# jspenmar/slowtv_monodepth

Hardware: AMD Instinct MI355X
Metric: training images/sec (640×192, 3-frame) at 1/2/4/8 MI355X; warp+SSIM HBM GB/s (higher is better)
Workload: dtype f32

## Files before the change

### slowtv_monodepth_amd/csrc/smd_conv_mfma.hip

```cpp
#include "smd_common.h"
#include "smd_kernels.h"
#include "smd_conv_mfma_dev.h"
#include <algorithm>

namespace smd {

template <typename T> __device__ __forceinline__ void store_out(T* p, size_t i, float v);
template <> __device__ __forceinline__ void store_out<float>(float* p, size_t i, float v) { p[i] = v; }
template <> __device__ __forceinline__ void store_out<bf16>(bf16* p, size_t i, float v) { p[i] = __float2bfloat16(v); }

template <int P>
__global__ __launch_bounds__(256) void k_conv_pack_w(const float* __restrict__ w, unsigned short* __restrict__ wp_fwd, unsigned short* __restrict__ wp_bwd, int CO, int C) {
  const int idx = blockIdx.x*256 + threadIdx.x;
  if (idx >= CO*C*9) return;
  const int tap = idx % 9, c = (idx/9) % C, co = idx/(9*C);
  unsigned pk[P];
  split_pair<P>(w[idx], 0.f, pk);
  if (wp_fwd) {
    const size_t base = ((((size_t)(co >> 5)*(C >> 4) + (c >> 4))*9 + tap)*P)*512 + (((c >> 3) & 1)*32 + (co & 31))*8 + (c & 7);
#pragma unroll
    for (int p = 0; p < P; ++p) wp_fwd[base + (size_t)p*512] = (unsigned short)(pk[p] & 0xffffu);
  }
  if (wp_bwd) {
    const size_t base = ((((size_t)(c >> 5)*(CO >> 4) + (co >> 4))*9 + (8 - tap))*P)*512 + (((co >> 3) & 1)*32 + (c & 31))*8 + (co & 7);
#pragma unroll
    for (int p = 0; p < P; ++p) wp_bwd[base + (size_t)p*512] = (unsigned short)(pk[p] & 0xffffu);
  }
}

#ifdef SMD_CONV_TRACE
__device__ unsigned long long g_conv_trace[8192][40];
#define SMD_CT(slot) do { if (wall == 0 && lid < 8192u && (slot) < 40) { const unsigned long long t_ = __builtin_amdgcn_s_memtime(); if (lane == 0) g_conv_trace[lid][(slot)] = t_; } } while (0)
#else
#define SMD_CT(slot) do { } while (0)
#endif
template <int TC> struct ConvTile {
  static constexpr int TRB = (TC == 64) ? 4 : 8;
  static constexpr int PW = TC + 2, PH = TRB + 2, NPIX = PW*PH;
};
template <> struct ConvTile<0> {
  static constexpr int TRB = 0, PW = 0, NPIX = 420;
};

template <int TC, int P, int OFF, typename TI, typename TO, int NM>
__global__ __launch_bounds__(256*NM, 2/NM) void k_conv_mfma(const TI* __restrict__ in_, const uint4* __restrict__ wp, TO* __restrict__ out,
                                                   int CK, int M, int hi, int wi, int ho, int wo, int KS, int kc_per_split, size_t split_stride,
                                                   unsigned gx, unsigned gy, unsigned gz, int S, int B) {
  using T = ConvTile<TC>;
  constexpr bool BAND = TC == 0;
  constexpr int NPIX = T::NPIX, off = OFF;
  const int PW = BAND ? wo + 2 : T::PW;
  constexpr bool ZERO = OFF != 0;
  constexpr int kBuf = P*NPIX*2;
  __shared__ uint4 tile[2*kBuf];
  const int lane = threadIdx.x & 63, wall = __builtin_amdgcn_readfirstlane(threadIdx.x >> 6), wv = wall & 3, mt = wall >> 2, j = lane & 31, g = lane >> 5;
  constexpr int NT = 256*NM;
  const int MG = M/(32*NM);
  const unsigned nblk = (unsigned)(MG*KS)*(BAND ? 1u : gx)*gy*gz, lid = xcd_block_id(nblk);
  if (lid >= nblk) return;
  const int mg = (int)(lid % MG)*NM + mt, ks = (lid/MG) % KS;
  const unsigned tl = lid/(MG*KS);
  const int BR = BAND ? (int)gx : 0, SEGP = (BR + 2)*PW;
  const int x0 = BAND ? 0 : (int)(tl % gx)*TC, y0 = BAND ? (int)(tl % gy)*BR : (int)((tl/gx) % gy)*T::TRB;
  const int b = BAND ? (int)(tl/gy)*S : (int)(tl/(gx*gy));
  const int KC = CK >> 4, kc0 = ks*kc_per_split, kc1 = min(KC, kc0 + kc_per_split);
  const size_t plane = (size_t)hi*wi;
  typedef typename RawOf<TI>::type R;
  const R* src = reinterpret_cast<const R*>(in_) + (size_t)b*CK*plane;
  auto band_pixel = [&](int nt, int& seg, int& ry, int& x) {
    const int p = (2*wv + nt)*32 + j, spx = BR*wo;
    seg = p/spx; const int q = p - seg*spx; ry = q/wo; x = q - ry*wo;
    if (seg >= S || b + seg >= B || y0 + ry >= ho) seg = -1;
  };
  int lbase[2] = {0, 0};
  if constexpr (BAND) {
#pragma unroll
    for (int nt = 0; nt < 2; ++nt) {
      int seg, ry, x;
      band_pixel(nt, seg, ry, x);
      lbase[nt] = seg >= 0 ? (seg*(BR + 2) + ry)*PW + x : 0;
    }
  }

  using Stage = PatchStager<NT, NPIX, P, R, ZERO>;
  constexpr int TRIPS = Stage::TRIPS;
  Stage stage;
  if constexpr (BAND) {
#pragma unroll
    for (int t = 0; t < TRIPS; ++t) {
      const int item = Stage::item(t), half = item >= NPIX ? 1 : 0, pix = item - half*NPIX;
      const int seg = pix/SEGP, rp = pix - seg*SEGP, r = rp/PW, cc = rp - r*PW;
      const int yy = y0 + r - off, xx = cc - off;
      const bool in_b = seg < S && b + seg < B;
      const int sofs = min(seg, B - 1 - b)*CK*(int)plane;
      if (ZERO) stage.pofs[t] = (in_b && yy >= 0 && yy < hi && xx >= 0 && xx < wi) ? sofs + yy*wi + xx : -1;
      else stage.pofs[t] = sofs + min(yy, hi - 1)*wi + min(xx, wi - 1);
    }
  } else stage.template rect_offsets<T::PW>(y0, x0, off, hi, wi);
  R v[TRIPS][8];
  auto request = [&](int kc) { stage.request(src, plane, kc, v); };
  auto file_trip = [&](int buf, int t) { stage.file_trip(tile, buf, t, v); };

  f32x16 acc[2], lo[2];
#pragma unroll
  for (int nt = 0; nt < 2; ++nt)
#pragma unroll
    for (int r = 0; r < 16; ++r) { acc[nt][r] = 0.f; lo[nt][r] = 0.f; }

  bf16x8 A[5][P], Bf[2][2][P];
  const uint4* wq = wp + ((size_t)mg*KC*9*P)*64 + lane;
  auto fetch_a = [&](bf16x8 (&dst)[P], int kc, int tap) {
#pragma unroll
    for (int p = 0; p < P; ++p) dst[p] = as_frag(wq[(size_t)((kc*9 + tap)*P + p)*64]);
  };
  auto read_b = [&](bf16x8 (&dst)[2][P], int buf, int tap) {
    const int ky = tap/3, kx = tap % 3;
#pragma unroll
    for (int nt = 0; nt < 2; ++nt) {
      const int r = (TC == 64) ? wv : 2*wv + nt, cb = (TC == 64) ? nt*32 : 0;
      Stage::read(tile, buf, BAND ? lbase[nt] + ky*PW + kx : (r + ky)*PW + cb + j + kx, g, dst[nt]);
    }
  };
  auto chunk = [&](int kc, int cur, auto more_tag) {
    constexpr bool MORE = decltype(more_tag)::value;
    [[maybe_unused]] const int cslot = 3 + 4*(kc - kc0);
    SMD_CT(cslot);
    read_b(Bf[0], cur, 0);
#pragma unroll
    for (int tap = 0; tap < 9; ++tap) {
      if (tap < 8) read_b(Bf[(tap + 1) & 1], cur, tap + 1);
      split_mfma<P>(A[tap % 5], Bf[tap & 1], acc, lo);
      if (tap <= 4) fetch_a(A[(tap + 4) % 5], kc, tap + 4);
      else if (MORE && tap >= 6) fetch_a(A[tap - 6], kc + 1, tap - 6);
      if (MORE && tap == 8) fetch_a(A[3], kc + 1, 3);
      if (MORE && tap == 4) request(kc + 1);
      if (MORE && tap >= 6) {
#pragma unroll
        for (int t = 0; t < TRIPS; ++t) if (t*3/TRIPS == tap - 6) file_trip(cur ^ 1, t);
      }
      __builtin_amdgcn_sched_barrier(0);
    }
    SMD_CT(cslot + 1);
    SMD_CT(cslot + 2);
    __syncthreads();
    SMD_CT(cslot + 3);
  };

  SMD_CT(0);
  if (kc0 < kc1) {
    request(kc0);
#pragma unroll
    for (int tap = 0; tap < 4; ++tap) fetch_a(A[tap], kc0, tap);
    stage.file(tile, 0, v);
  }
  SMD_CT(1);
  __syncthreads();
  SMD_CT(2);
  int kc = kc0;
  for (; kc + 1 < kc1; ++kc) chunk(kc, (kc - kc0) & 1, std::true_type{});
  if (kc < kc1) chunk(kc, (kc - kc0) & 1, std::false_type{});
  float* dstf = reinterpret_cast<float*>(out) + (size_t)ks*split_stride;
#pragma unroll
  for (int nt = 0; nt < 2; ++nt) {
    int y, x, bo = b;
    bool ok;
    if constexpr (BAND) {
      int seg, ry;
      band_pixel(nt, seg, ry, x);
      ok = seg >= 0; y = y0 + ry; bo = b + seg;
    } else {
      const int r = (TC == 64) ? wv : 2*wv + nt, cb = (TC == 64) ? nt*32 : 0;
      y = y0 + r; x = x0 + cb + j; ok = y < ho && x < wo;
    }
    if (ok) {
#pragma unroll
      for (int rr = 0; rr < 16; ++rr) {
        const int m = mg*32 + mfma32_row(rr, g);
        const size_t o = (((size_t)bo*M + m)*ho + y)*wo + x;
        if (KS > 1) dstf[o] = acc[nt][rr] + lo[nt][rr];
        else store_out<TO>(out, o, acc[nt][rr] + lo[nt][rr]);
      }
    }
  }
  SMD_CT(39);
}

typedef float f32x4u __attribute__((ext_vector_type(4), aligned(4)));

template <int P>
__global__ __launch_bounds__(256) void k_conv_pack_w16(const float* __restrict__ w, unsigned short* __restrict__ wp_fwd, unsigned short* __restrict__ wp_bwd, int C) {
  const int idx = blockIdx.x*256 + threadIdx.x;
  const int nslots = (C >> 4)*5*64*8;
  if (idx < nslots && wp_fwd) {
    const int e = idx & 7, lane = (idx >> 3) & 63, s = (idx >> 9) % 5, ch = idx/(512*5);
    const int j = lane & 15, q = lane >> 4, tap = 2*s + (q >> 1), k = 16*ch + 8*(q & 1) + e;
    unsigned pk[P];
    split_pair<P>(tap < 9 ? w[((size_t)j*C + k)*9 + tap] : 0.f, 0.f, pk);
#pragma unroll
    for (int p = 0; p < P; ++p) wp_fwd[(((size_t)(ch*5 + s)*P + p)*64 + lane)*8 + e] = (unsigned short)(pk[p] & 0xffffu);
  }
  if (idx < 5*64*8 && wp_bwd && C == 16) {
    const int e = idx & 7, lane = (idx >> 3) & 63, s = idx >> 9;
    const int j = lane & 15, q = lane >> 4, tap = 2*s + (q >> 1), k = 8*(q & 1) + e;
    unsigned pk[P];
    split_pair<P>(tap < 9 ? w[((size_t)k*C + j)*9 + (8 - tap)] : 0.f, 0.f, pk);
#pragma unroll
    for (int p = 0; p < P; ++p) wp_bwd[(((size_t)s*P + p)*64 + lane)*8 + e] = (unsigned short)(pk[p] & 0xffffu);
  }
}

template <int NCH, int P, bool BWD, typename TI, typename TO>
__global__ __launch_bounds__(256) void k_conv16_mfma(const TI* __restrict__ in_, const uint4* __restrict__ wp, TO* __restrict__ out,
                                                     int hi, int wi, int ho, int wo, unsigned gx, unsigned gy, unsigned gz) {
  using T = ConvTile<64>;
  constexpr int NPIX = T::NPIX, PW = T::PW, off = BWD ? 2 : 0, CK = 16*NCH;
  __shared__ uint4 tile[P*NPIX*2];
  const int lane = threadIdx.x & 63, wv = __builtin_amdgcn_readfirstlane(threadIdx.x >> 6), i = lane & 15, q = lane >> 4;
  const unsigned nblk = gx*gy*gz, lid = xcd_block_id(nblk);
  if (lid >= nblk) return;
  const int x0 = (int)(lid % gx)*64, y0 = (int)((lid/gx) % gy)*4, b = (int)(lid/(gx*gy));
  const size_t plane = (size_t)hi*wi;
  typedef typename RawOf<TI>::type R;
  const R* src = reinterpret_cast<const R*>(in_) + (size_t)b*CK*plane;

  bf16x8 Wr[NCH][5][P];
#pragma unroll
  for (int ch = 0; ch < NCH; ++ch)
#pragma unroll
    for (int s = 0; s < 5; ++s)
#pragma unroll
      for (int p = 0; p < P; ++p) Wr[ch][s][p] = as_frag(wp[((ch*5 + s)*P + p)*64 + lane]);

  using Stage = PatchStager<256, NPIX, P, R, BWD>;
  constexpr int ITEMS = Stage::ITEMS, TRIPS = Stage::TRIPS;
  int pofs[TRIPS];
#pragma unroll
  for (int t = 0; t < TRIPS; ++t) {
    const int item = min(t*256 + (int)threadIdx.x, ITEMS - 1);
    const int half = item >= NPIX ? 1 : 0, pix = item - half*NPIX;
    const int r = pix/PW, cc = pix - r*PW;
    const int yy = y0 + r - off, xx = x0 + cc - off;
    if (BWD) pofs[t] = (yy >= 0 && yy < hi && xx >= 0 && xx < wi) ? yy*wi + xx : -1;
    else pofs[t] = min(yy, hi - 1)*wi + min(xx, wi - 1);
  }
  int dpix[5];
#pragma unroll
  for (int s = 0; s < 5; ++s) { const int tq = min(2*s + (q >> 1), 8); dpix[s] = (tq/3)*PW + tq % 3; }

  f32x4v acc[4], lo[4];
#pragma unroll
  for (int r = 0; r < 4; ++r) { acc[r] = f32x4v{0.f, 0.f, 0.f, 0.f}; lo[r] = f32x4v{0.f, 0.f, 0.f, 0.f}; }

#pragma unroll
  for (int ch = 0; ch < NCH; ++ch) {
    R v[TRIPS][8];
#pragma unroll
    for (int t = 0; t < TRIPS; ++t) {
      const int item = min(t*256 + (int)threadIdx.x, ITEMS - 1);
      const int half = item >= NPIX ? 1 : 0;
      const R* p = src + (size_t)(ch*16 + half*8)*plane + (size_t)max(pofs[t], 0);
#pragma unroll
      for (int e = 0; e < 8; ++e) v[t][e] = (!BWD || pofs[t] >= 0) ? p[(size_t)e*plane] : R(0);
    }
    if (ch > 0) __syncthreads();
#pragma unroll
    for (int t = 0; t < TRIPS; ++t) {
      const int item = t*256 + (int)threadIdx.x;
      if (item < ITEMS) {
        const int half = item >= NPIX ? 1 : 0, pix = item - half*NPIX;
        unsigned pk[4][P];
#pragma unroll
        for (int k = 0; k < 4; ++k) split_pair<P>(v[t][2*k], v[t][2*k + 1], pk[k]);
        const int slot = patch_slot(pix, half);
#pragma unroll
        for (int p = 0; p < P; ++p) tile[p*NPIX*2 + slot] = uint4{pk[0][p], pk[1][p], pk[2][p], pk[3][p]};
      }
    }
    __syncthreads();
#pragma unroll
    for (int s = 0; s < 5; ++s) {
#pragma unroll
      for (int r = 0; r < 4; ++r) {
        bf16x8 A[P];
        Stage::read(tile, 0, r*PW + 16*wv + i + dpix[s], q & 1, A);
        split_mfma<P>(A, Wr[ch][s], acc[r], lo[r]);
      }
    }
  }
  const int x = x0 + 16*wv + 4*q;
#pragma unroll
  for (int r = 0; r < 4; ++r) {
    const int y = y0 + r;
    if (y >= ho || x >= wo) continue;
    TO* dstp = out + (((size_t)b*16 + i)*ho + y)*wo + x;
    const f32x4v o = acc[r] + lo[r];
    if constexpr (sizeof(TO) == 4) {
      if (x + 3 < wo) *reinterpret_cast<f32x4u*>(dstp) = o;
      else { dstp[0] = o[0]; if (x + 1 < wo) dstp[1] = o[1]; if (x + 2 < wo) dstp[2] = o[2]; }
    } else {
      const unsigned lo2 = pack_bf16_rne(o[0], o[1]), hi2 = pack_bf16_rne(o[2], o[3]);
      if (x + 3 < wo && (wo & 1) == 0) { reinterpret_cast<unsigned*>(dstp)[0] = lo2; reinterpret_cast<unsigned*>(dstp)[1] = hi2; }
      else {
        unsigned short* d16 = reinterpret_cast<unsigned short*>(dstp);
        d16[0] = (unsigned short)(lo2 & 0xffffu);
        if (x + 1 < wo) d16[1] = (unsigned short)(lo2 >> 16);
        if (x + 2 < wo) d16[2] = (unsigned short)(hi2 & 0xffffu);
        if (x + 3 < wo) d16[3] = (unsigned short)(hi2 >> 16);
      }
    }
  }
}

template <typename TO>
__global__ __launch_bounds__(256) void k_conv_split_sum(const float* __restrict__ part, TO* __restrict__ out, size_t n4, int KS) {
  const size_t i = (size_t)blockIdx.x*256 + threadIdx.x;
  if (i >= n4) return;
  const f4* p = reinterpret_cast<const f4*>(part);
  f4 s = p[i];
  for (int k = 1; k < KS; ++k) s += p[(size_t)k*n4 + i];
  if constexpr (sizeof(TO) == 4) reinterpret_cast<f4*>(out)[i] = s;
  else { unsigned* o = reinterpret_cast<unsigned*>(out) + 2*i; o[0] = pack_bf16_rne(s.x, s.y); o[1] = pack_bf16_rne(s.z, s.w); }
}

static size_t thin_packed_elems(int C, int pieces) { return (size_t)(C >> 4)*5*pieces*512; }
size_t conv_mfma_packed_elems(int C, int CO, int pieces) { return std::max((size_t)CO*C*9*pieces, CO == 16 ? thin_packed_elems(C, pieces) : (size_t)0); }

#define SMD_BY_PIECES(pieces, CALL) do { if ((pieces) == 3) { CALL(3, float); } else if ((pieces) == 2) { CALL(2, float); } else { CALL(1, bf16); } } while (0)

template <int P, typename T>
static void launch_conv16(const void* in, const void* wp, void* out, int B, int CK, bool bwd, int hi, int wi, int ho, int wo, hipStream_t st) {
  const unsigned gx = ceil_div(wo, 64), gy = ceil_div(ho, 4), gz = B;
  const dim3 grid(8*(unsigned)ceil_div((long long)gx*gy*gz, 8ll));
  const uint4* wq = (const uint4*)wp;
  const T* i_ = (const T*)in; T* o_ = (T*)out;
  if (bwd) hipLaunchKernelGGL((k_conv16_mfma<1, P, true, T, T>), grid, dim3(256), 0, st, i_, wq, o_, hi, wi, ho, wo, gx, gy, gz);
  else if (CK == 16) hipLaunchKernelGGL((k_conv16_mfma<1, P, false, T, T>), grid, dim3(256), 0, st, i_, wq, o_, hi, wi, ho, wo, gx, gy, gz);
  else hipLaunchKernelGGL((k_conv16_mfma<2, P, false, T, T>), grid, dim3(256), 0, st, i_, wq, o_, hi, wi, ho, wo, gx, gy, gz);
}

hipError_t launch_conv_mfma_pack(const float* w, void* wp_fwd, void* wp_bwd, int C, int CO, int pieces, hipStream_t st) {
  if (CO == 16) {
    void* thin_bwd = (C == 16) ? wp_bwd : nullptr;
    if (wp_fwd || thin_bwd) {
      const dim3 g16(ceil_div((C >> 4)*5*512, 256));
#define SMD_CALL(P, T) hipLaunchKernelGGL((k_conv_pack_w16<P>), g16, dim3(256), 0, st, w, (unsigned short*)wp_fwd, (unsigned short*)thin_bwd, C)
      SMD_BY_PIECES(pieces, SMD_CALL);
#undef SMD_CALL
    }
    if (C == 16 || !wp_bwd) return hipGetLastError();
    wp_fwd = nullptr;
  }
  const dim3 grid(ceil_div(CO*C*9, 256));
#define SMD_CALL(P, T) hipLaunchKernelGGL((k_conv_pack_w<P>), grid, dim3(256), 0, st, w, (unsigned short*)wp_fwd, (unsigned short*)wp_bwd, CO, C)
  SMD_BY_PIECES(pieces, SMD_CALL);
#undef SMD_CALL
  return hipGetLastError();
}

struct ConvShape { int TC, TRB, NM, KS, kcs, S; unsigned gx, gy, gz; dim3 grid; size_t out_elems; };
static double band_shape(int B, int CK, int ho, int wo, int& BR, int& S) {
  constexpr int NP = ConvTile<0>::NPIX;
  const int PW = wo + 2;
  if (3*PW > NP || (long long)B*CK*(ho + 2)*PW >= (1ll << 31)) return 0.0;
  if (ho*wo <= 128) {
    BR = ho; S = std::min(256/(ho*wo), B);
    while (S > 1 && S*(ho + 2)*PW > NP) --S;
  } else {
    S = 1; BR = std::min(ho, 256/wo);
    while (BR > 0 && (BR + 2)*PW > NP) --BR;
    if (BR == 0) return 0.0;
  }
  return (double)B*ho*wo/((double)ceil_div(ho, BR)*ceil_div(B, S)*256.0);
}
static ConvShape conv_shape(int B, int CK, int M, int ho, int wo, bool two_tiles) {
  ConvShape s;
  s.TC = wo >= 48 ? 64 : 32; s.TRB = wo >= 48 ? 4 : 8; s.S = 1;
  const int KC = CK >> 4;
  {
    const double rect = (double)B*ho*wo/((double)ceil_div(wo, s.TC)*s.TC*ceil_div(ho, s.TRB)*s.TRB*B);
    int BR = 0, S = 1;
    const double band = rect < 0.9 ? band_shape(B, CK, ho, wo, BR, S) : 0.0;
    if (band > rect + 0.05) {
      s.TC = 0; s.TRB = BR; s.S = S; s.NM = 1;
      s.gx = BR; s.gy = ceil_div(ho, BR); s.gz = ceil_div(B, S);
      s.out_elems = (size_t)B*M*ho*wo;
      const long long base = (long long)s.gy*s.gz*(M/32);
      double best = -1.0;
      for (int kcs = std::min(2, KC); kcs <= KC; ++kcs) {
        const int KS = ceil_div(KC, kcs);
        if (ceil_div(KC, KS) != kcs) continue;
        const double cost = (double)ceil_div(base*KS, 512ll)*(kcs + 1) + (KS > 1 ? (2.0*KS + 1.0)*s.out_elems*4.0/25e6 : 0.0);
        if (best < 0.0 || cost < best - 1e-9) { best = cost; s.kcs = kcs; s.KS = KS; }
      }
      s.grid = dim3(8*(unsigned)ceil_div(base*s.KS, 8ll));
      return s;
    }
  }
  const long long tiles = (long long)ceil_div(wo, s.TC)*ceil_div(ho, s.TRB)*B;
  s.NM = (M % 64 == 0 && tiles*(M/64) >= 256 && two_tiles) ? 2 : 1;
  const long long base = tiles*(M/(32*s.NM));
  int ks = 1;
  if (base < 384) ks = (int)std::min<long long>(std::max(KC/2, 1), (512 + base - 1)/base);
  s.kcs = ceil_div(KC, ks); s.KS = ceil_div(KC, s.kcs);
  s.gx = ceil_div(wo, s.TC); s.gy = ceil_div(ho, s.TRB); s.gz = B;
  s.grid = dim3(8*(unsigned)ceil_div((long long)s.gx*s.gy*s.gz*(M/(32*s.NM))*s.KS, 8ll));
  s.out_elems = (size_t)B*M*ho*wo;
  return s;
}
size_t conv_mfma_split_elems(ConvOp op, bool zpad, int B, int C, int CO, int h, int w, bool two_tiles) {
  if (op == ConvOp::Wgt || !conv_mfma_served(op, zpad, C, CO) || (CO == 16 && (op == ConvOp::Fwd || C == 16))) return 0;
  const int e = zpad ? 0 : 2;
  const ConvShape s = op == ConvOp::Fwd ? conv_shape(B, C, CO, h, w, two_tiles) : conv_shape(B, CO, C, h + e, w + e, two_tiles);
  return s.KS > 1 ? (size_t)s.KS*s.out_elems : 0;
}

template <int P, int OFF, typename T>
static void launch_conv_form(const void* in, const void* wp, void* out, float* split_ws, int B, int CK, int M, int hi, int wi, int ho, int wo, bool two_tiles, hipStream_t st) {
  const ConvShape s = conv_shape(B, CK, M, ho, wo, two_tiles);
  const uint4* wq = (const uint4*)wp;
  const T* i_ = (const T*)in;
  T* dst = s.KS > 1 ? reinterpret_cast<T*>(split_ws) : (T*)out;
  if (s.TC == 0) hipLaunchKernelGGL((k_conv_mfma<0, P, OFF, T, T, 1>), s.grid, dim3(256), 0, st, i_, wq, dst, CK, M, hi, wi, ho, wo, s.KS, s.kcs, s.out_elems, s.gx, s.gy, s.gz, s.S, B);
  else if (s.NM == 2) {
    if (s.TC == 64) hipLaunchKernelGGL((k_conv_mfma<64, P, OFF, T, T, 2>), s.grid, dim3(512), 0, st, i_, wq, dst, CK, M, hi, wi, ho, wo, s.KS, s.kcs, s.out_elems, s.gx, s.gy, s.gz, 1, B);
    else hipLaunchKernelGGL((k_conv_mfma<32, P, OFF, T, T, 2>), s.grid, dim3(512), 0, st, i_, wq, dst, CK, M, hi, wi, ho, wo, s.KS, s.kcs, s.out_elems, s.gx, s.gy, s.gz, 1, B);
  } else if (s.TC == 64) hipLaunchKernelGGL((k_conv_mfma<64, P, OFF, T, T, 1>), s.grid, dim3(256), 0, st, i_, wq, dst, CK, M, hi, wi, ho, wo, s.KS, s.kcs, s.out_elems, s.gx, s.gy, s.gz, 1, B);
  else hipLaunchKernelGGL((k_conv_mfma<32, P, OFF, T, T, 1>), s.grid, dim3(256), 0, st, i_, wq, dst, CK, M, hi, wi, ho, wo, s.KS, s.kcs, s.out_elems, s.gx, s.gy, s.gz, 1, B);
  if (s.KS > 1) {
    const size_t n4 = s.out_elems/4;
    hipLaunchKernelGGL((k_conv_split_sum<T>), dim3((unsigned)((n4 + 255)/256)), dim3(256), 0, st, split_ws, (T*)out, n4, s.KS);
  }
}

#define SMD_BY_PIECES_F32(pieces, CALL) do { if ((pieces) == 3) { CALL(3); } else { CALL(2); } } while (0)
hipError_t launch_conv_mfma_fwd(const void* x, const void* wp_fwd, void* y, float* split_ws, bool zpad, int B, int C, int CO, int h, int w, int pieces, bool two_tiles, hipStream_t st) {
  if (zpad) {
#define SMD_CALL(P) launch_conv_form<P, 1, float>(x, wp_fwd, y, split_ws, B, C, CO, h, w, h, w, two_tiles, st)
    SMD_BY_PIECES_F32(pieces, SMD_CALL);
#undef SMD_CALL
  } else if (CO == 16) {
#define SMD_CALL(P, T) launch_conv16<P, T>(x, wp_fwd, y, B, C, false, h + 2, w + 2, h, w, st)
    SMD_BY_PIECES(pieces, SMD_CALL);
#undef SMD_CALL
  } else {
#define SMD_CALL(P, T) launch_conv_form<P, 0, T>(x, wp_fwd, y, split_ws, B, C, CO, h + 2, w + 2, h, w, two_tiles, st)
    SMD_BY_PIECES(pieces, SMD_CALL);
#undef SMD_CALL
  }
  return hipGetLastError();
}
hipError_t launch_conv_mfma_bwd_data(const void* gy, const void* wp_bwd, void* g_x, float* split_ws, bool zpad, int B, int C, int CO, int h, int w, int pieces, bool two_tiles, hipStream_t st) {
  if (zpad) {
#define SMD_CALL(P) launch_conv_form<P, 1, float>(gy, wp_bwd, g_x, split_ws, B, CO, C, h, w, h, w, two_tiles, st)
    SMD_BY_PIECES_F32(pieces, SMD_CALL);
#undef SMD_CALL
  } else if (CO == 16 && C == 16) {
#define SMD_CALL(P, T) launch_conv16<P, T>(gy, wp_bwd, g_x, B, 16, true, h, w, h + 2, w + 2, st)
    SMD_BY_PIECES(pieces, SMD_CALL);
#undef SMD_CALL
  } else {
#define SMD_CALL(P, T) launch_conv_form<P, 2, T>(gy, wp_bwd, g_x, split_ws, B, CO, C, h, w, h + 2, w + 2, two_tiles, st)
    SMD_BY_PIECES(pieces, SMD_CALL);
#undef SMD_CALL
  }
  return hipGetLastError();
}

}

#ifdef SMD_CONV_TRACE
extern "C" int smd_debug_conv_trace(unsigned long long* host_out, int blocks) {
  return (int)hipMemcpyFromSymbol(host_out, HIP_SYMBOL(smd::g_conv_trace), (size_t)blocks*40*sizeof(unsigned long long), 0, hipMemcpyDeviceToHost);
}
#endif
```

Before: 963.6.

## Stage conv weight packing through LDS and emit coalesced 16-byte stores

The weight-pack kernel is rewritten so each block owns a 16-input-channel by 16/32-output-channel tile. It loads weight pairs, splits them into bf16 pieces, and assembles the packed forward and transposed backward images in padded shared memory. It then writes them out as contiguous uint4 stores instead of scattered 2-byte stores per element. This targets the uncoalesced global writes of the per-step weight repack, at the cost of more shared memory, fixed assumptions about tile sizes, and a more intricate indexing scheme. It only affects a small packing kernel within the training step.

```diff
diff --git a/slowtv_monodepth_amd/csrc/smd_conv_mfma.hip b/slowtv_monodepth_amd/csrc/smd_conv_mfma.hip
--- a/slowtv_monodepth_amd/csrc/smd_conv_mfma.hip
+++ b/slowtv_monodepth_amd/csrc/smd_conv_mfma.hip
@@ -9,22 +9,58 @@
 template <> __device__ __forceinline__ void store_out<float>(float* p, size_t i, float v) { p[i] = v; }
 template <> __device__ __forceinline__ void store_out<bf16>(bf16* p, size_t i, float v) { p[i] = __float2bfloat16(v); }
 
+constexpr int kPackThreads = 384, kPackQuads = 3;
+constexpr int kPackFwdSlab = 256 + 4, kPackBwdSlab = 128 + 4;
 template <int P>
-__global__ __launch_bounds__(256) void k_conv_pack_w(const float* __restrict__ w, unsigned short* __restrict__ wp_fwd, unsigned short* __restrict__ wp_bwd, int CO, int C) {
-  const int idx = blockIdx.x*256 + threadIdx.x;
-  if (idx >= CO*C*9) return;
-  const int tap = idx % 9, c = (idx/9) % C, co = idx/(9*C);
-  unsigned pk[P];
-  split_pair<P>(w[idx], 0.f, pk);
+__global__ __launch_bounds__(kPackThreads) void k_conv_pack_w(const float* __restrict__ w, uint4* __restrict__ wp_fwd, uint4* __restrict__ wp_bwd, int CO, int C, int RCO) {
+  __shared__ uint4 img_f[9*P*kPackFwdSlab/4], img_b[2*9*P*kPackBwdSlab/4];
+  unsigned* lf = reinterpret_cast<unsigned*>(img_f);
+  unsigned* lb = reinterpret_cast<unsigned*>(img_b);
+  const int tid = threadIdx.x, KCF = C >> 4, KCB = CO >> 4;
+  const int c0 = (int)(blockIdx.x % KCF)*16, co0 = (int)(blockIdx.x/KCF)*RCO;
+  const int nquads = (RCO >> 1)*72, NKB = RCO >> 4;
+  const size_t row = (size_t)C*9;
+  float v[kPackQuads][4];
+#pragma unroll
+  for (int t = 0; t < kPackQuads; ++t) {
+    const int q = t*kPackThreads + tid;
+    if (q < nquads) {
+      const int tap = q % 9, c = ((q/9) & 7)*2, co = (q/72)*2;
+      const float* s = w + (size_t)(co0 + co)*row + (size_t)(c0 + c)*9 + tap;
+      v[t][0] = s[0]; v[t][1] = s[9]; v[t][2] = s[row]; v[t][3] = s[row + 9];
+    }
+  }
+#pragma unroll
+  for (int t = 0; t < kPackQuads; ++t) {
+    const int q = t*kPackThreads + tid;
+    if (q < nquads) {
+      const int tap = q % 9, c = ((q/9) & 7)*2, co = (q/72)*2;
+      unsigned r0[P], r1[P];
+      split_pair<P>(v[t][0], v[t][1], r0);
+      split_pair<P>(v[t][2], v[t][3], r1);
+      if (wp_fwd) {
+        const int at = ((c >> 3)*32 + co)*4 + ((c & 7) >> 1);
+#pragma unroll
+        for (int p = 0; p < P; ++p) { unsigned* d = lf + (tap*P + p)*kPackFwdSlab + at; d[0] = r0[p]; d[4] = r1[p]; }
+      }
+      if (wp_bwd) {
+        const int k = co & 15, at = ((k >> 3)*16 + c)*4 + ((k & 7) >> 1);
+#pragma unroll
+        for (int p = 0; p < P; ++p) {
+          unsigned* d = lb + (((co >> 4)*9 + 8 - tap)*P + p)*kPackBwdSlab + at;
+          d[0] = (r0[p] & 0xffffu) | (r1[p] << 16); d[4] = (r0[p] >> 16) | (r1[p] & 0xffff0000u);
+        }
+      }
+    }
+  }
+  __syncthreads();
   if (wp_fwd) {
-    const size_t base = ((((size_t)(co >> 5)*(C >> 4) + (c >> 4))*9 + tap)*P)*512 + (((c >> 3) & 1)*32 + (co & 31))*8 + (c & 7);
-#pragma unroll
-    for (int p = 0; p < P; ++p) wp_fwd[base + (size_t)p*512] = (unsigned short)(pk[p] & 0xffffu);
+    uint4* dst = wp_fwd + ((size_t)(co0 >> 5)*KCF + (c0 >> 4))*(9*P*64);
+    for (int i = tid; i < 9*P*64; i += kPackThreads) dst[i] = img_f[(i >> 6)*(kPackFwdSlab/4) + (i & 63)];
   }
   if (wp_bwd) {
-    const size_t base = ((((size_t)(c >> 5)*(CO >> 4) + (co >> 4))*9 + (8 - tap))*P)*512 + (((co >> 3) & 1)*32 + (c & 31))*8 + (co & 7);
-#pragma unroll
-    for (int p = 0; p < P; ++p) wp_bwd[base + (size_t)p*512] = (unsigned short)(pk[p] & 0xffffu);
+    uint4* dst = wp_bwd + ((size_t)(c0 >> 5)*KCB + (co0 >> 4))*(9*P*64) + (c0 & 16);
+    for (int i = tid; i < NKB*9*P*32; i += kPackThreads) dst[(i >> 5)*64 + ((i >> 4) & 1)*32 + (i & 15)] = img_b[(i >> 5)*(kPackBwdSlab/4) + (i & 31)];
   }
 }
 
@@ -350,8 +386,9 @@
     if (C == 16 || !wp_bwd) return hipGetLastError();
     wp_fwd = nullptr;
   }
-  const dim3 grid(ceil_div(CO*C*9, 256));
-#define SMD_CALL(P, T) hipLaunchKernelGGL((k_conv_pack_w<P>), grid, dim3(256), 0, st, w, (unsigned short*)wp_fwd, (unsigned short*)wp_bwd, CO, C)
+  const int RCO = CO % 32 == 0 ? 32 : 16;
+  const dim3 grid((unsigned)((C >> 4)*(CO/RCO)));
+#define SMD_CALL(P, T) hipLaunchKernelGGL((k_conv_pack_w<P>), grid, dim3(kPackThreads), 0, st, w, (uint4*)wp_fwd, (uint4*)wp_bwd, CO, C, RCO)
   SMD_BY_PIECES(pieces, SMD_CALL);
 #undef SMD_CALL
   return hipGetLastError();
```

Result: slower. 931.8 (-3.3%).
